# jklebes/MetropolisEngine

Hardware: AMD Instinct MI355X
Metric: MC steps/sec (chains x sweeps) at 2^20 chains, 16 params (higher is better)
Workload: dtype f64

## Files before the change

metropolisengine_amd/csrc/me_device.h:

```cpp
#pragma once

#include <type_traits>
#include <utility>

#include <hip/hip_runtime.h>
#include <stdint.h>

#include "me_internal.h"
#include "me_math64.h"

namespace me {

struct U4 {
  uint32_t x, y, z, w;
};

__device__ __forceinline__ uint32_t xor3(uint32_t a, uint32_t b, uint32_t c) {
  return __builtin_amdgcn_bitop3_b32(a, b, c, 0x96);
}
__device__ __forceinline__ U4 philox4x32_10(U4 c, uint32_t k0, uint32_t k1) {
#pragma unroll
  for (int r = 0; r < 10; ++r) {
    const uint64_t p0 = (uint64_t)0xD2511F53u * c.x;
    const uint64_t p1 = (uint64_t)0xCD9E8D57u * c.z;
    U4 n;
    n.x = xor3((uint32_t)(p1 >> 32), c.y, k0);
    n.y = (uint32_t)p1;
    n.z = xor3((uint32_t)(p0 >> 32), c.w, k1);
    n.w = (uint32_t)p0;
    c = n;
    k0 += 0x9E3779B9u;
    k1 += 0xBB67AE85u;
  }
  return c;
}
__device__ __forceinline__ U4 philox_counter(unsigned long long gid, unsigned long long step, int b) {
  U4 ctr;
  ctr.x = (uint32_t)gid;
  ctr.y = (uint32_t)(gid >> 32);
  ctr.z = (uint32_t)step;
  ctr.w = ((uint32_t)(step >> 32) << 16) | (uint32_t)b;
  return ctr;
}
__device__ __forceinline__ U4 philox_block(unsigned long long gid, unsigned long long step, int b, uint32_t seed_lo, uint32_t seed_hi) {
  return philox4x32_10(philox_counter(gid, step, b), seed_lo, seed_hi);
}

__device__ __forceinline__ float fma_(float a, float b, float c) { return __builtin_fmaf(a, b, c); }
__device__ __forceinline__ double fma_(double a, double b, double c) { return __builtin_fma(a, b, c); }

template <typename R>
struct Num;

template <>
struct Num<float> {
  static __device__ __forceinline__ void prepare() {}
  static __device__ __forceinline__ float unit(uint32_t w) {
    return __builtin_fmaf((float)w, 2.3283064365386963e-10f, 1.1641532182693481e-10f);
  }
  static __device__ __forceinline__ void normal_pair(uint32_t wa, uint32_t wb, float &g0, float &g1) {
    const float u1 = unit(wa), u2 = unit(wb);
    const float r = __builtin_amdgcn_sqrtf(-1.3862943611198906f * __builtin_amdgcn_logf(u1));
    g0 = r * __builtin_amdgcn_cosf(u2);
    g1 = r * __builtin_amdgcn_sinf(u2);
  }
  static __device__ __forceinline__ bool uphill(float u, float d, float, float inv_temp_log2e) {
    return u <= __builtin_amdgcn_exp2f(-d * inv_temp_log2e);
  }
  static __device__ __forceinline__ float adapt(float w, bool acc, float ratio, float p, float damping,
                                                float up, float down) {
    return __builtin_fmaf(w, acc ? up : down, w);
  }
  static __device__ __forceinline__ float sqrt_(float v) { return __builtin_sqrtf(v); }
  static __device__ __forceinline__ float abs_(float v) { return __builtin_fabsf(v); }
  static __device__ __forceinline__ bool finite(float v) { return __builtin_isfinite(v); }
};

template <>
struct Num<double> {
  static __device__ __forceinline__ double (*log_table())[2] {
    __shared__ __attribute__((aligned(16))) double table[math64::kLogEntries][2];
    return table;
  }
  static __device__ __forceinline__ void prepare() {
    double(*table)[2] = log_table();
    for (int k0 = threadIdx.x; k0 < math64::kLogEntries; k0 += 2 * (int)blockDim.x) {
      const int k1 = k0 + (int)blockDim.x;
      const bool second = k1 < math64::kLogEntries;
      const double a0 = math64::kLogTable[k0][0], a1 = math64::kLogTable[k0][1];
      const double b0 = second ? math64::kLogTable[k1][0] : 0.0, b1 = second ? math64::kLogTable[k1][1] : 0.0;
      table[k0][0] = a0;
      table[k0][1] = a1;
      if (second) {
        table[k1][0] = b0;
        table[k1][1] = b1;
      }
    }
    __syncthreads();
  }
  static __device__ __forceinline__ double unit(uint32_t w) { return ((double)w + 0.5) * (1.0 / 4294967296.0); }
  static __device__ __forceinline__ void normal_pair(uint32_t wa, uint32_t wb, double &g0, double &g1) {
    math64::normal_pair(wa, wb, log_table(), g0, g1);
  }
  static __device__ __forceinline__ bool uphill(double u, double d, double inv_temp, double) {
    return u <= math64::exp_nonpos(-d * inv_temp);
  }
  static __device__ __forceinline__ double adapt(double w, bool acc, double ratio, double p, double damping,
                                                 double, double) {
    const double scale = w * ratio;
    return acc ? w + scale * (1.0 - p) / damping : w - scale * p / damping;
  }
  static __device__ __forceinline__ double sqrt_(double v) { return sqrt(v); }
  static __device__ __forceinline__ double abs_(double v) { return fabs(v); }
  static __device__ __forceinline__ bool finite(double v) { return isfinite(v); }
};

#ifndef ME_NT_AUX
#define ME_NT_AUX 2
#endif
template <typename R>
struct Field {
  __amdgpu_buffer_rsrc_t rsrc;
  unsigned int row_bytes;
  __device__ __forceinline__ Field(const R *base, long long n, int rows)
      : rsrc(__builtin_amdgcn_make_buffer_rsrc(const_cast<R *>(base), 0, (unsigned int)(rows * n * (long long)sizeof(R)),
                                               0x00020000)),
        row_bytes((unsigned int)(n * (long long)sizeof(R))) {}
  __device__ __forceinline__ R load(int row, unsigned int chain_off) const {
    if constexpr (sizeof(R) == 4) {
      return __builtin_bit_cast(R, __builtin_amdgcn_raw_buffer_load_b32(rsrc, chain_off, (unsigned int)row * row_bytes, 0));
    } else {
      const auto v = __builtin_amdgcn_raw_buffer_load_b64(rsrc, chain_off, (unsigned int)row * row_bytes, 0);
      return __builtin_bit_cast(R, v);
    }
  }
  __device__ __forceinline__ R load_nt(int row, unsigned int chain_off) const {
    if constexpr (sizeof(R) == 4) {
      return __builtin_bit_cast(R, __builtin_amdgcn_raw_buffer_load_b32(rsrc, chain_off, (unsigned int)row * row_bytes, ME_NT_AUX));
    } else {
      const auto v = __builtin_amdgcn_raw_buffer_load_b64(rsrc, chain_off, (unsigned int)row * row_bytes, ME_NT_AUX);
      return __builtin_bit_cast(R, v);
    }
  }
  __device__ __forceinline__ void store_nt(int row, unsigned int chain_off, R value) const {
    if constexpr (sizeof(R) == 4) {
      __builtin_amdgcn_raw_buffer_store_b32(__builtin_bit_cast(unsigned int, value), rsrc, chain_off,
                                            (unsigned int)row * row_bytes, ME_NT_AUX);
    } else {
      using v2 = decltype(__builtin_amdgcn_raw_buffer_load_b64(rsrc, 0u, 0u, 0));
      __builtin_amdgcn_raw_buffer_store_b64(__builtin_bit_cast(v2, value), rsrc, chain_off,
                                            (unsigned int)row * row_bytes, ME_NT_AUX);
    }
  }
  __device__ __forceinline__ void store(int row, unsigned int chain_off, R value) const {
    if constexpr (sizeof(R) == 4) {
      __builtin_amdgcn_raw_buffer_store_b32(__builtin_bit_cast(unsigned int, value), rsrc, chain_off,
                                            (unsigned int)row * row_bytes, 0);
    } else {
      using v2 = decltype(__builtin_amdgcn_raw_buffer_load_b64(rsrc, 0u, 0u, 0));
      __builtin_amdgcn_raw_buffer_store_b64(__builtin_bit_cast(v2, value), rsrc, chain_off,
                                            (unsigned int)row * row_bytes, 0);
    }
  }
};

template <typename R>
__device__ __forceinline__ R chain_energy(const Field<R> &fe, unsigned int chain_off, int n_terms) {
  R e = fe.load(0, chain_off);
  for (int t = 1; t < n_terms; ++t) e = e + fe.load(t, chain_off);
  return e;
}

template <typename R>
__device__ __forceinline__ unsigned int tiled_offset(long long c, int entries) {
  return (unsigned int)(((c >> 6) * (long long)entries * 64 + (c & 63)) * (long long)sizeof(R));
}
template <typename R>
struct TiledField {
  __amdgpu_buffer_rsrc_t rsrc;
  __device__ __forceinline__ TiledField(const R *base, long long n, int entries)
      : rsrc(__builtin_amdgcn_make_buffer_rsrc(const_cast<R *>(base), 0,
                                               (unsigned int)(((n + 63) >> 6) * (long long)entries * 64 * (long long)sizeof(R)),
                                               0x00020000)) {}
  static constexpr unsigned int kEntryBytes = 64u * (unsigned int)sizeof(R);
  template <int AUX>
  __device__ __forceinline__ R load_aux(int k, unsigned int tile_off) const {
    if constexpr (sizeof(R) == 4) {
      return __builtin_bit_cast(R, __builtin_amdgcn_raw_buffer_load_b32(rsrc, tile_off, (unsigned int)k * kEntryBytes, AUX));
    } else {
      const auto v = __builtin_amdgcn_raw_buffer_load_b64(rsrc, tile_off, (unsigned int)k * kEntryBytes, AUX);
      return __builtin_bit_cast(R, v);
    }
  }
  template <int AUX>
  __device__ __forceinline__ void store_aux(int k, unsigned int tile_off, R value) const {
    if constexpr (sizeof(R) == 4) {
      __builtin_amdgcn_raw_buffer_store_b32(__builtin_bit_cast(unsigned int, value), rsrc, tile_off, (unsigned int)k * kEntryBytes, AUX);
    } else {
      using v2 = decltype(__builtin_amdgcn_raw_buffer_load_b64(rsrc, 0u, 0u, 0));
      __builtin_amdgcn_raw_buffer_store_b64(__builtin_bit_cast(v2, value), rsrc, tile_off, (unsigned int)k * kEntryBytes, AUX);
    }
  }
  __device__ __forceinline__ R load(int k, unsigned int tile_off) const { return load_aux<0>(k, tile_off); }
  __device__ __forceinline__ R load_nt(int k, unsigned int tile_off) const { return load_aux<ME_NT_AUX>(k, tile_off); }
  __device__ __forceinline__ void store(int k, unsigned int tile_off, R value) const { store_aux<0>(k, tile_off, value); }
  __device__ __forceinline__ void store_nt(int k, unsigned int tile_off, R value) const { store_aux<ME_NT_AUX>(k, tile_off, value); }
};

template <bool NT, class F>
__device__ __forceinline__ auto packed_load(const F &f, int row, unsigned int chain_off) {
  if constexpr (NT) return f.load_nt(row, chain_off);
  else return f.load(row, chain_off);
}
template <bool NT, class F, typename R>
__device__ __forceinline__ void packed_store(const F &f, int row, unsigned int chain_off, R value) {
  if constexpr (NT) f.store_nt(row, chain_off, value);
  else f.store(row, chain_off, value);
}

template <typename R, bool NTS>
struct StateField : Field<R> {
  using Field<R>::Field;
  __device__ __forceinline__ R load(int row, unsigned int chain_off) const {
    if constexpr (NTS) return Field<R>::load_nt(row, chain_off);
    else return Field<R>::load(row, chain_off);
  }
  __device__ __forceinline__ void store(int row, unsigned int chain_off, R value) const {
    if constexpr (NTS) Field<R>::store_nt(row, chain_off, value);
    else Field<R>::store(row, chain_off, value);
  }
};

#ifndef ME_TILED_STATE_DOF
#define ME_TILED_STATE_DOF 16
#endif
constexpr int kTiledStateDof = ME_TILED_STATE_DOF;
template <typename R, int D, bool NTS = false>
struct XField {
  static constexpr bool kTiled = D >= kTiledStateDof;
  std::conditional_t<kTiled, TiledField<R>, StateField<R, NTS>> f;
  __device__ __forceinline__ XField(const R *base, long long n) : f(base, n, D) {}
  static __device__ __forceinline__ unsigned int offset(long long c) {
    if constexpr (kTiled) return tiled_offset<R>(c, D);
    else return (unsigned int)c * (unsigned int)sizeof(R);
  }
  __device__ __forceinline__ R load(int row, unsigned int off) const {
    if constexpr (kTiled && NTS) return f.load_nt(row, off);
    else return f.load(row, off);
  }
  __device__ __forceinline__ void store(int row, unsigned int off, R value) const {
    if constexpr (kTiled && NTS) f.store_nt(row, off, value);
    else f.store(row, off, value);
  }
};
template <typename R, int D>
__device__ __forceinline__ long long state_index(long long c, int row, long long n) {
  if constexpr (D >= kTiledStateDof) return ((c >> 6) * (long long)D + row) * 64 + (c & 63);
  else return (long long)row * n + c;
}

constexpr int kMaxPackedInRegisters = 160;
#ifndef ME_STREAM_F64_ENTRIES
#define ME_STREAM_F64_ENTRIES 96
#endif
constexpr int kStreamF64Entries = ME_STREAM_F64_ENTRIES;

template <typename R, int NR, int NC>
struct EnergyIso {
  static constexpr int D = NR + 2 * NC;
  R a;
  __device__ __forceinline__ R operator()(const R (&x)[D]) const {
    R s0 = 0, s1 = 0;
#pragma unroll
    for (int d = 0; d + 1 < D; d += 2) {
      s0 += x[d] * x[d];
      s1 += x[d + 1] * x[d + 1];
    }
    if constexpr (D % 2 == 1) s0 += x[D - 1] * x[D - 1];
    return a * (s0 + s1);
  }
};

template <typename R, int NR, int NC>
struct EnergyDiag {
  static constexpr int D = NR + 2 * NC;
  R w[D];
  __device__ __forceinline__ R operator()(const R (&x)[D]) const {
    R s0 = 0, s1 = 0;
#pragma unroll
    for (int d = 0; d + 1 < D; d += 2) {
      s0 += w[d] * x[d] * x[d];
      s1 += w[d + 1] * x[d + 1] * x[d + 1];
    }
    if constexpr (D % 2 == 1) s0 += w[D - 1] * x[D - 1] * x[D - 1];
    return s0 + s1;
  }
};

template <typename R, int NR, int NC>
struct EnergyDense {
  static constexpr int D = NR + 2 * NC;
  static constexpr int PT = D * (D + 1) / 2;
  const R *a;
  static __device__ __forceinline__ R *folded() {
    __shared__ R t[PT];
    return t;
  }
  __device__ __forceinline__ void prepare() const {
    R *t = folded();
    constexpr int kBatch = 8;
    for (int k0 = threadIdx.x; k0 < PT; k0 += kBatch * (int)blockDim.x) {
      R lo[kBatch], hi[kBatch];
#pragma unroll
      for (int u = 0; u < kBatch; ++u) {
        const int k = k0 + u * (int)blockDim.x;
        lo[u] = hi[u] = R(0);
        if (k < PT) {
          int i = (int)((__builtin_sqrtf((float)(8 * k + 1)) - 1.0f) * 0.5f);
          if ((i + 1) * (i + 2) / 2 <= k) ++i;
          if (i * (i + 1) / 2 > k) --i;
          const int j = k - i * (i + 1) / 2;
          lo[u] = a[i * D + j];
          if (i != j) hi[u] = a[j * D + i];
        }
      }
#pragma unroll
      for (int u = 0; u < kBatch; ++u) {
        const int k = k0 + u * (int)blockDim.x;
        if (k < PT) t[k] = lo[u] + hi[u];
      }
    }
    __syncthreads();
  }
  __device__ __forceinline__ R operator()(const R (&x)[D]) const {
    const R *t = folded();
    asm volatile("" ::: "memory");
    R e = 0;
#pragma unroll
    for (int i = 0; i < D; ++i) {
      R y = 0;
#pragma unroll
      for (int j = 0; j <= i; ++j) y += t[i * (i + 1) / 2 + j] * x[j];
      e += x[i] * y;
    }
    return e;
  }
};

template <typename R, int NR, int NC>
struct EnergyLandau {
  static constexpr int D = NR + 2 * NC;
  R k, alpha, beta;
  __device__ __forceinline__ R operator()(const R (&x)[D]) const {
    static_assert(NR == 2 && NC == 1, "Landau toy is 2 real + 1 complex");
    const R a2 = fma_(x[2], x[2], x[3] * x[3]);
    const R ox = R(1) - x[0], oy = R(1) - x[1];
    return fma_(x[0] * x[1], fma_(beta * a2, a2, alpha * a2), fma_(k * ox, ox, k * oy * oy));
  }
};

template <typename R, int NR, int NC>
struct EnergyCylinder {
  static constexpr int D = NR + 2 * NC;
  R kappa, gamma, wavenumber;
  __device__ __forceinline__ R operator()(const R (&x)[D]) const {
    static_assert(NR >= 1 && NC >= 1, "cylinder surrogate needs an amplitude and a field");
    R s = 0;
#pragma unroll
    for (int i = 0; i < NR; ++i) s += x[i] * x[i];
    const R x0 = x[0];
    const R surface = kappa * s / (R(1) - x0 * x0);
    const R amp = R(1) + R(0.5) * x0 * x0;
    R field = 0, tot = 0;
#pragma unroll
    for (int j = 0; j < NC; ++j) {
      const R q = wavenumber * (R(j) - R(NC - 1) * R(0.5));
      const R mod2 = fma_(x[NR + j], x[NR + j], x[NR + NC + j] * x[NR + NC + j]);
      field += (gamma + q * q * amp) * mod2;
      tot += mod2;
    }
    return surface + field + R(0.5) * tot * tot;
  }
};

template <typename R, int NR, int NC>
struct EnergyLandauTerms {
  static constexpr int D = NR + 2 * NC;
  static constexpr int kTerms = 2;
  R k, alpha, beta;
  static constexpr unsigned term_groups(int t) { return t == 0 ? 3u : 1u; }
  __device__ __forceinline__ R term(int t, const R (&x)[D]) const {
    static_assert(NR == 2 && NC == 1, "Landau toy is 2 real + 1 complex");
    if (t == 0) {
      const R a2 = fma_(x[2], x[2], x[3] * x[3]);
      return x[0] * x[1] * fma_(beta * a2, a2, alpha * a2);
    }
    const R ox = R(1) - x[0], oy = R(1) - x[1];
    return fma_(k * ox, ox, k * oy * oy);
  }
};

template <class E, typename R, int D>
__device__ __forceinline__ auto energy_reject(const E &en, const R (&x)[D], int) -> decltype(en.reject(x)) {
  return en.reject(x);
}
template <class E, typename R, int D>
__device__ __forceinline__ bool energy_reject(const E &, const R (&)[D], long) {
  return false;
}

template <class E>
__device__ __forceinline__ auto energy_prepare(const E &en, int) -> decltype(en.prepare()) {
  en.prepare();
}
template <class E>
__device__ __forceinline__ void energy_prepare(const E &, long) {}

template <class E, class = void>
struct term_count { static constexpr int value = 1; };
template <class E>
struct term_count<E, std::void_t<decltype(E::kTerms)>> { static constexpr int value = E::kTerms; };

template <typename R, class Energy, int GROUP>
struct EnergyLedger {
  static constexpr int T = term_count<Energy>::value;
  R term[T];
  static constexpr bool moves(int t) {
    if constexpr (T == 1 || GROUP == GROUP_ALL) return true;
    else return (Energy::term_groups(t) & (GROUP == GROUP_REAL ? 1u : 2u)) != 0u;
  }
  template <class F>
  __device__ __forceinline__ void load(const F &fe, unsigned int coff) {
#pragma unroll
    for (int t = 0; t < T; ++t)
      if (moves(t)) term[t] = fe.load(t, coff);
  }
  template <class F>
  __device__ __forceinline__ void store(const F &fe, unsigned int coff) const {
#pragma unroll
    for (int t = 0; t < T; ++t)
      if (moves(t)) fe.store(t, coff, term[t]);
  }
  __device__ __forceinline__ R partial() const {
    R s = 0;
    bool first = true;
#pragma unroll
    for (int t = 0; t < T; ++t)
      if (moves(t)) {
        s = first ? term[t] : s + term[t];
        first = false;
      }
    return s;
  }
  template <int D>
  __device__ __forceinline__ R propose(const Energy &en, const R (&xp)[D], R (&out)[T]) const {
    if constexpr (T == 1) {
      out[0] = en(xp);
      return out[0];
    } else {
      R s = 0;
      bool first = true;
#pragma unroll
      for (int t = 0; t < T; ++t)
        if (moves(t)) {
          out[t] = en.term(t, xp);
          s = first ? out[t] : s + out[t];
          first = false;
        }
      return s;
    }
  }
  __device__ __forceinline__ void commit(bool accept, const R (&out)[T]) {
#pragma unroll
    for (int t = 0; t < T; ++t)
      if (moves(t)) term[t] = accept ? out[t] : term[t];
  }
};

template <typename R>
struct StepArgs {
  R *x, *energy, *width;
  const R *factor;
  const R *inj_normals;
  const R *inj_uniforms;
  unsigned long long *accept_slots;
  unsigned int *status;
  long long n;
  unsigned long long chain_offset, step_index;
  uint32_t seed_lo, seed_hi;
  int n_sweeps, reject_kind;
  int split_widths;
  int stale_total;
  R reject_bound, temp, inv_temp, inv_temp_log2e, ratio, p, damping, up, down;
  const R *ladder;
  int tiles_per_rung;
};

template <typename R>
StepArgs<R> typed(const StepLaunch &l) {
  StepArgs<R> a;
  a.x = (R *)l.x;
  a.energy = (R *)l.energy;
  a.width = (R *)l.width;
  a.factor = (const R *)l.factor;
  a.inj_normals = (const R *)l.inj_normals;
  a.inj_uniforms = (const R *)l.inj_uniforms;
  a.accept_slots = l.accept_slots;
  a.status = l.status;
  a.n = l.n;
  a.chain_offset = l.chain_offset;
  a.step_index = l.step_index;
  a.seed_lo = (uint32_t)l.seed;
  a.seed_hi = (uint32_t)(l.seed >> 32);
  a.n_sweeps = l.n_sweeps;
  a.reject_kind = l.reject_kind;
  a.split_widths = l.split_widths;
  a.stale_total = l.stale_total;
  a.reject_bound = (R)l.reject_bound;
  a.temp = (R)l.temp;
  a.inv_temp = l.temp > 0 ? (R)(1.0 / l.temp) : (R)0;
  a.inv_temp_log2e = l.temp > 0 ? (R)(1.4426950408889634 / l.temp) : (R)0;
  a.ratio = (R)l.ratio;
  a.p = (R)l.target_acceptance;
  a.damping = (R)l.damping;
  a.up = (R)(l.ratio * (1.0 - l.target_acceptance) / l.damping);
  a.down = (R)(-l.ratio * l.target_acceptance / l.damping);
  a.ladder = (const R *)l.ladder;
  a.tiles_per_rung = l.tiles_per_rung;
  return a;
}

template <typename R>
__device__ __forceinline__ void publish_step(const StepArgs<R> &a, unsigned int waves, unsigned int wave_accepted, bool bad_energy,
                                             bool bad_width, bool bad_pivot = false) {
  if ((threadIdx.x & 63) == 0 && wave_accepted) {
    unsigned long long *slot = a.accept_slots + (size_t)blockIdx.x * waves + (threadIdx.x >> 6);
    *slot += (unsigned long long)wave_accepted;
  }
  const unsigned int bits = (bad_energy ? ST_NONFINITE_ENERGY : 0u) | (bad_width ? ST_BAD_WIDTH : 0u) | (bad_pivot ? ST_BAD_PIVOT : 0u);
  if (bits) atomicOr(a.status, bits);
}

template <bool LADDER, typename R>
__device__ __forceinline__ bool uphill_at(const StepArgs<R> &a, long long c, R u, R diff) {
  if constexpr (!LADDER) {
    return a.temp > R(0) && Num<R>::uphill(u, diff, a.inv_temp, a.inv_temp_log2e);
  } else {
    const int rung = __builtin_amdgcn_readfirstlane((int)(c >> 6)) / a.tiles_per_rung;
    return Num<R>::uphill(u, diff, a.ladder[2 * rung], a.ladder[2 * rung + 1]);
  }
}

__host__ __device__ constexpr int tri(int i, int j) { return i * (i + 1) / 2 + j; }
__host__ __device__ constexpr int cre(int pr, int i, int j) { return pr + i * i + 2 * j; }
__host__ __device__ constexpr int cim(int pr, int i, int j) { return pr + i * i + 2 * j + 1; }
__host__ __device__ constexpr int cdiag(int pr, int i) { return pr + i * i + 2 * i; }

template <class F, int... I>
__device__ __forceinline__ void static_for_impl(F &&fn, std::integer_sequence<int, I...>) {
  (fn(std::integral_constant<int, I>{}), ...);
}
template <int N, class F>
__device__ __forceinline__ void static_for(F &&fn) {
  static_for_impl(fn, std::make_integer_sequence<int, N>{});
}
__host__ __device__ constexpr unsigned long long join_halves(int hi, int lo) {
  return ((unsigned long long)(unsigned int)hi << 32) | (unsigned long long)(unsigned int)lo;
}
static_assert(join_halves(0x00007f12, (int)0x80000000u) == 0x00007f1280000000ull, "low half with bit 31 set must not sign-extend");
static_assert(join_halves((int)0xffff8000u, (int)0xfffffff0u) == 0xffff8000fffffff0ull, "both halves are zero-extended");
#ifndef ME_STREAM_CHUNK_BYTES
#define ME_STREAM_CHUNK_BYTES 128
#endif

template <typename R, int NR, int NC, bool INJECT>
__device__ __forceinline__ void draw_step(const StepArgs<R> &a, long long c, unsigned long long gid, int s,
                                          R (&g)[2 * ((NR + 2 * NC + 1) / 2)], R &u) {
  constexpr int D = NR + 2 * NC;
  constexpr int NW = 2 * ((D + 1) / 2);
  constexpr int NBLK = (NW + 1 + 3) / 4;
  using N_ = Num<R>;
  [[maybe_unused]] const unsigned long long step = a.step_index + (unsigned long long)s;
  if constexpr (INJECT) {
#pragma unroll
    for (int j = 0; j < D; ++j) g[j] = a.inj_normals[((long long)s * D + j) * a.n + c];
    u = a.inj_uniforms[(long long)s * a.n + c];
  } else {
    uint32_t words[4 * NBLK];
#pragma unroll
    for (int b = 0; b < NBLK; ++b) {
      const U4 o = philox_block(gid, step, b, a.seed_lo, a.seed_hi);
      words[4 * b + 0] = o.x;
      words[4 * b + 1] = o.y;
      words[4 * b + 2] = o.z;
      words[4 * b + 3] = o.w;
    }
#pragma unroll
    for (int q = 0; q < NW / 2; ++q) N_::normal_pair(words[2 * q], words[2 * q + 1], g[2 * q], g[2 * q + 1]);
    u = N_::unit(words[NW]);
  }

}

template <typename R, int NR, int NC, int CK, int GROUP, class Fac>
__device__ __forceinline__ void propose_registers(const R (&x)[NR + 2 * NC], const R (&g)[2 * ((NR + 2 * NC + 1) / 2)], R w_r, R w_c,
                                                  Fac &&fac, R (&xp)[NR + 2 * NC]) {
  constexpr int D = NR + 2 * NC;
  [[maybe_unused]] constexpr int PR = NR * (NR + 1) / 2;
  constexpr bool MOVE_REAL = NR > 0 && GROUP != GROUP_COMPLEX;
  constexpr bool MOVE_COMPLEX = NC > 0 && GROUP != GROUP_REAL;
#pragma unroll
  for (int d = 0; d < D; ++d) xp[d] = x[d];
  if constexpr (CK == CK_IDENTITY) {
    if constexpr (MOVE_REAL) {
#pragma unroll
      for (int i = 0; i < NR; ++i) xp[i] = x[i] + w_r * g[i];
    }
    if constexpr (MOVE_COMPLEX) {
#pragma unroll
      for (int j = 0; j < NC; ++j) {
        xp[NR + j] = x[NR + j] + w_c * (g[NR + j] * R(0.70710678118654752440));
        xp[NR + NC + j] = x[NR + NC + j] + w_c * (g[NR + NC + j] * R(0.70710678118654752440));
      }
    }
  } else {
    if constexpr (MOVE_REAL) {
#pragma unroll
      for (int i = 0; i < NR; ++i) {
        R acc = 0;
#pragma unroll
        for (int j = 0; j <= i; ++j) acc += fac(tri(i, j)) * g[j];
        xp[i] = x[i] + w_r * acc;
      }
    }
    if constexpr (MOVE_COMPLEX) {
#pragma unroll
      for (int i = 0; i < NC; ++i) {
        R are = 0, aim = 0;
#pragma unroll
        for (int j = 0; j < i; ++j) {
          const R lre = fac(cre(PR, i, j));
          const R lim = fac(cim(PR, i, j));
          const R wre = g[NR + j] * R(0.70710678118654752440), wim = g[NR + NC + j] * R(0.70710678118654752440);
          are += lre * wre - lim * wim;
          aim += lre * wim + lim * wre;
        }
        const R ld = fac(cdiag(PR, i));
        are += ld * (g[NR + i] * R(0.70710678118654752440));
        aim += ld * (g[NR + NC + i] * R(0.70710678118654752440));
        xp[NR + i] = x[NR + i] + w_c * are;
        xp[NR + NC + i] = x[NR + NC + i] + w_c * aim;
      }
    }
  }

}

template <typename R, int NR, int NC, class Energy, int CK, int GROUP, bool LADDER, class Ledger>
__device__ __forceinline__ void decide_step(const StepArgs<R> &a, long long c, const Energy &en, bool stale_total, R u,
                                            const R (&g)[2 * ((NR + 2 * NC + 1) / 2)], R (&x)[NR + 2 * NC], const R (&xp)[NR + 2 * NC],
                                            Ledger &ledger, R &total_q5, R &w, R &w_r, R &w_c, unsigned int &wave_accepted,
                                            bool &bad_energy) {
  [[maybe_unused]] constexpr int D = NR + 2 * NC;
  constexpr bool MOVE_REAL = NR > 0 && GROUP != GROUP_COMPLEX;
  constexpr bool MOVE_COMPLEX = NC > 0 && GROUP != GROUP_REAL;
  using N_ = Num<R>;
  bool rejected = false;
  if (a.reject_kind == ME_REJECT_ABS_REAL0_GE) rejected = !(N_::abs_(xp[0]) < a.reject_bound);
  else if (a.reject_kind == ME_REJECT_USER) rejected = energy_reject(en, xp, 0);
  R terms_new[Ledger::T];
  const R e_new = ledger.propose(en, xp, terms_new);
  const R diff = e_new - (stale_total ? total_q5 : ledger.partial());
  bool accept = diff <= R(0);
  if constexpr (LADDER) accept = accept || uphill_at<true>(a, c, u, diff);
  else if (a.temp > R(0)) accept = accept || N_::uphill(u, diff, a.inv_temp, a.inv_temp_log2e);
  accept = accept && !rejected;
  bad_energy |= (!rejected && !N_::finite(e_new));
  if constexpr (CK == CK_IDENTITY) {
    const R wa_r = accept ? w_r : R(0), wa_c = accept ? w_c : R(0);
    if constexpr (MOVE_REAL) {
#pragma unroll
      for (int i = 0; i < NR; ++i) x[i] = x[i] + wa_r * g[i];
    }
    if constexpr (MOVE_COMPLEX) {
#pragma unroll
      for (int j = 0; j < NC; ++j) {
        x[NR + j] = x[NR + j] + wa_c * (g[NR + j] * R(0.70710678118654752440));
        x[NR + NC + j] = x[NR + NC + j] + wa_c * (g[NR + NC + j] * R(0.70710678118654752440));
      }
    }
  } else {
#pragma unroll
    for (int d = 0; d < D; ++d) x[d] = accept ? xp[d] : x[d];
  }
  if (stale_total) total_q5 = accept ? e_new : total_q5;
  else ledger.commit(accept, terms_new);
  w = N_::adapt(w, accept, a.ratio, a.p, a.damping, a.up, a.down);
  if constexpr (GROUP == GROUP_ALL) w_r = w_c = w;
  else if constexpr (GROUP == GROUP_REAL) w_r = w;
  else w_c = w;
  wave_accepted += (unsigned int)__popcll(__ballot(accept));
}

template <typename R, int NR, int NC, class Energy, int CK, bool INJECT, int GROUP, bool LADDER, class Ledger, class Fac>
__device__ __forceinline__ void run_sweeps(const StepArgs<R> &a, const Energy &en, long long c, unsigned long long gid,
                                           bool stale_total, R (&x)[NR + 2 * NC], Ledger &ledger, R &total_q5, R &w, R &w_r,
                                           R &w_c, Fac &&fac, unsigned int &wave_accepted, bool &bad_energy) {
  constexpr int D = NR + 2 * NC;
  constexpr int NW = 2 * ((D + 1) / 2);
  for (int s = 0; s < a.n_sweeps; ++s) {
    R g[NW], u, xp[D];
    draw_step<R, NR, NC, INJECT>(a, c, gid, s, g, u);
    propose_registers<R, NR, NC, CK, GROUP>(x, g, w_r, w_c, fac, xp);
    decide_step<R, NR, NC, Energy, CK, GROUP, LADDER>(a, c, en, stale_total, u, g, x, xp, ledger, total_q5, w, w_r, w_c, wave_accepted, bad_energy);
  }
}

#ifndef ME_STEP_WAVES_PER_EU
#define ME_STEP_WAVES_PER_EU 0
#endif
#if ME_STEP_WAVES_PER_EU > 0
#define ME_STEP_BOUNDS __launch_bounds__(kFusedStepThreads, ME_STEP_WAVES_PER_EU)
#else
#define ME_STEP_BOUNDS __launch_bounds__(kFusedStepThreads)
#endif

#ifndef ME_STEP_PRIO_SHIFT
#define ME_STEP_PRIO_SHIFT 8
#endif
__device__ __forceinline__ void stagger_priority() {
#if ME_STEP_PRIO_SHIFT >= 0
  switch ((blockIdx.x >> ME_STEP_PRIO_SHIFT) & 3u) {
    case 0: __builtin_amdgcn_s_setprio(3); break;
    case 1: __builtin_amdgcn_s_setprio(2); break;
    case 2: __builtin_amdgcn_s_setprio(1); break;
    default: break;
  }
#endif
}

template <typename R, int NR, int NC, class Energy, int CK, bool INJECT = false, int GROUP = GROUP_ALL, bool NTS = false,
          bool LADDER = false>
__global__ void ME_STEP_BOUNDS k_step(StepArgs<R> a, Energy en) {
  constexpr int D = NR + 2 * NC;
  constexpr bool MIXED = NR > 0 && NC > 0;
  static_assert(GROUP == GROUP_ALL || MIXED, "group-wise kernels exist for mixed engines only");
  using N_ = Num<R>;

  stagger_priority();
  if constexpr (!INJECT) N_::prepare();
  energy_prepare(en, 0);
  unsigned int wave_accepted = 0;
  bool bad_energy = false, bad_width = false;
  const long long stride = (long long)gridDim.x * blockDim.x;
  using Ledger = EnergyLedger<R, Energy, GROUP>;
  const XField<R, D, NTS> fx(a.x, a.n);
  const StateField<R, NTS> fe(a.energy, a.n, Ledger::T + (MIXED ? 1 : 0)), fw(a.width, a.n, MIXED ? 3 : 1);
  const bool stale_total = MIXED && GROUP == GROUP_ALL && a.stale_total != 0;
  constexpr bool PER_CHAIN = CK == CK_PER_CHAIN || CK == CK_PER_CHAIN_NT;
  constexpr int PF = PER_CHAIN ? NR * (NR + 1) / 2 + NC * NC : 0;
  constexpr bool STREAM_FACTOR = PER_CHAIN && (PF > kMaxPackedInRegisters ||
                                               (!INJECT && sizeof(R) == 8 && NC == 0 && PF > kStreamF64Entries));
  const TiledField<R> ffac(a.factor, a.n, STREAM_FACTOR ? 0 : PF);
  for (long long c = (long long)blockIdx.x * blockDim.x + threadIdx.x; c < a.n; c += stride) {
    const unsigned int coff = (unsigned int)c * (unsigned int)sizeof(R);
    const unsigned int xoff = fx.offset(c);
    R x[D];
#pragma unroll
    for (int d = 0; d < D; ++d) x[d] = fx.load(d, xoff);
    Ledger ledger;
    R total_q5 = R(0);
    if (stale_total) total_q5 = fe.load(Ledger::T, coff);
    else ledger.load(fe, coff);
    R w = fw.load(MIXED ? GROUP : 0, coff);
    R w_r = w, w_c = w;
    if constexpr (MIXED && GROUP == GROUP_ALL) {
      if (a.split_widths) {
        w_r = fw.load(GROUP_REAL, coff);
        w_c = fw.load(GROUP_COMPLEX, coff);
      }
    }
    const unsigned long long gid = a.chain_offset + (unsigned long long)c;
    [[maybe_unused]] const unsigned int toff = tiled_offset<R>(c, PF);
    auto fac = [&](int k) -> R {
      if constexpr (CK == CK_PER_CHAIN_NT) return ffac.load_nt(k, toff);
      else if constexpr (CK == CK_PER_CHAIN) return ffac.load(k, toff);
      else return a.factor[k];
    };

    if constexpr (STREAM_FACTOR) {
      constexpr int NW = 2 * ((D + 1) / 2);
      for (int s = 0; s < a.n_sweeps; ++s) {
        static_assert(!INJECT, "the streamed-factor form has no replay hook");
        constexpr int NBLK = (NW + 1 + 3) / 4;
        const unsigned long long step = a.step_index + (unsigned long long)s;
        R g[NW];
        R u_accept;
        {
          uint32_t words[4 * NBLK];
#pragma unroll
          for (int b = 0; b < NBLK; ++b) {
            const U4 o = philox_block(gid, step, b, a.seed_lo, a.seed_hi);
            words[4 * b + 0] = o.x;
            words[4 * b + 1] = o.y;
            words[4 * b + 2] = o.z;
            words[4 * b + 3] = o.w;
          }
#pragma unroll
          for (int q = 0; q < NW / 2; ++q) N_::normal_pair(words[2 * q], words[2 * q + 1], g[2 * q], g[2 * q + 1]);
          u_accept = N_::unit(words[NW]);
        }
        R xp[D];
#pragma unroll
        for (int d = 0; d < D; ++d) xp[d] = x[d];
        asm volatile("" ::: "memory");
        constexpr int CH = (int)(ME_STREAM_CHUNK_BYTES / sizeof(R));
        const R *tile_base = a.factor + (c >> 6) * (long long)PF * 64;
        const unsigned long long tb = (unsigned long long)tile_base;
        const R *tile_uniform = (const R *)join_halves(__builtin_amdgcn_readfirstlane((int)(tb >> 32)),
                                                       __builtin_amdgcn_readfirstlane((int)(unsigned int)tb));
        const __amdgpu_buffer_rsrc_t tile = __builtin_amdgcn_make_buffer_rsrc(const_cast<R *>(tile_uniform), 0,
                                                                               (unsigned int)(PF * 64 * sizeof(R)), 0x00020000);
        const unsigned int lane_off = (unsigned int)(c & 63) * (unsigned int)sizeof(R);
        auto entry = [&](int k) -> R {
          constexpr int AUX = CK == CK_PER_CHAIN_NT ? ME_NT_AUX : 0;
          if constexpr (sizeof(R) == 4)
            return __builtin_bit_cast(R, __builtin_amdgcn_raw_buffer_load_b32(tile, lane_off, (unsigned int)k * 64u * 4u, AUX));
          else
            return __builtin_bit_cast(R, __builtin_amdgcn_raw_buffer_load_b64(tile, lane_off, (unsigned int)k * 64u * 8u, AUX));
        };
        R f[2][CH];
#pragma unroll
        for (int u = 0; u < CH; ++u)
          if (u < PF) f[0][u] = entry(u);
        auto use = [&](auto entry_index) -> R {
          constexpr int k = decltype(entry_index)::value;
          if constexpr (k % CH == 0) {
            __builtin_amdgcn_sched_barrier(0);
#pragma unroll
            for (int u = 0; u < CH; ++u)
              if (k + CH + u < PF) f[(k / CH + 1) & 1][u] = entry(k + CH + u);
            __builtin_amdgcn_sched_barrier(0);
          }
          return f[(k / CH) & 1][k % CH];
        };
        static_for<NR>([&](auto row_index) {
          constexpr int i = decltype(row_index)::value;
          R acc = 0;
          static_for<i + 1>([&](auto col_index) {
            constexpr int j = decltype(col_index)::value, k = tri(i, j);
            const R l = use(std::integral_constant<int, k>{});
            acc = j == 0 ? l * g[0] : acc + l * g[j];
          });
          if constexpr (GROUP != GROUP_COMPLEX) xp[i] = x[i] + w_r * acc;
        });
        static_for<NC>([&](auto row_index) {
          constexpr int i = decltype(row_index)::value;
          R are = 0, aim = 0;
          static_for<i>([&](auto col_index) {
            constexpr int j = decltype(col_index)::value;
            const R lre = use(std::integral_constant<int, cre(NR * (NR + 1) / 2, i, j)>{});
            const R lim = use(std::integral_constant<int, cim(NR * (NR + 1) / 2, i, j)>{});
            const R wre = g[NR + j] * R(0.70710678118654752440), wim = g[NR + NC + j] * R(0.70710678118654752440);
            are += lre * wre - lim * wim;
            aim += lre * wim + lim * wre;
          });
          const R ld = use(std::integral_constant<int, cdiag(NR * (NR + 1) / 2, i)>{});
          are += ld * (g[NR + i] * R(0.70710678118654752440));
          aim += ld * (g[NR + NC + i] * R(0.70710678118654752440));
          if constexpr (GROUP != GROUP_REAL) {
            xp[NR + i] = x[NR + i] + w_c * are;
            xp[NR + NC + i] = x[NR + NC + i] + w_c * aim;
          }
        });
        bool rejected = false;
        if (a.reject_kind == ME_REJECT_ABS_REAL0_GE) rejected = !(N_::abs_(xp[0]) < a.reject_bound);
        else if (a.reject_kind == ME_REJECT_USER) rejected = energy_reject(en, xp, 0);
        R terms_new[Ledger::T];
        const R e_new = ledger.propose(en, xp, terms_new);
        const R diff = e_new - (stale_total ? total_q5 : ledger.partial());
        bool accept = diff <= R(0);
        if constexpr (LADDER) accept = accept || uphill_at<true>(a, c, u_accept, diff);
        else if (a.temp > R(0)) accept = accept || N_::uphill(u_accept, diff, a.inv_temp, a.inv_temp_log2e);
        accept = accept && !rejected;
        bad_energy |= (!rejected && !N_::finite(e_new));
#pragma unroll
        for (int d = 0; d < D; ++d) x[d] = accept ? xp[d] : x[d];
        if (stale_total) total_q5 = accept ? e_new : total_q5;
        else ledger.commit(accept, terms_new);
        w = N_::adapt(w, accept, a.ratio, a.p, a.damping, a.up, a.down);
        if constexpr (GROUP == GROUP_ALL) w_r = w_c = w;
        else if constexpr (GROUP == GROUP_REAL) w_r = w;
        else w_c = w;
        wave_accepted += (unsigned int)__popcll(__ballot(accept));
      }
    } else {
      run_sweeps<R, NR, NC, Energy, CK, INJECT, GROUP, LADDER>(a, en, c, gid, stale_total, x, ledger, total_q5, w, w_r, w_c, fac, wave_accepted, bad_energy);
    }
    bad_width |= !(w > R(0));
#pragma unroll
    for (int d = 0; d < D; ++d) fx.store(d, xoff, x[d]);
    if (stale_total) fe.store(Ledger::T, coff, total_q5);
    else ledger.store(fe, coff);
    fw.store(MIXED ? GROUP : 0, coff, w);
  }
  publish_step(a, blockDim.x >> 6, wave_accepted, bad_energy, bad_width);
}

template <typename R, int NR, int NC, class Energy>
__global__ void __launch_bounds__(kStepThreads) k_init_energy(const R *xs, R *energy, long long n, unsigned int *status,
                                                                Energy en, int total_row) {
  constexpr int D = NR + 2 * NC;
  energy_prepare(en, 0);
  const long long stride = (long long)gridDim.x * kStepThreads;
  for (long long c = (long long)blockIdx.x * kStepThreads + threadIdx.x; c < n; c += stride) {
    R x[D];
#pragma unroll
    for (int d = 0; d < D; ++d) x[d] = xs[state_index<R, D>(c, d, n)];
    constexpr int T = term_count<Energy>::value;
    bool finite = true;
    R total = R(0);
#pragma unroll
    for (int t = 0; t < T; ++t) {
      R e;
      if constexpr (T == 1) e = en(x);
      else e = en.term(t, x);
      energy[(long long)t * n + c] = e;
      total = t == 0 ? e : total + e;
      finite = finite && Num<R>::finite(e);
    }
    if (total_row >= 0) energy[(long long)total_row * n + c] = total;
    if (!finite) atomicOr(status, (unsigned int)ST_NONFINITE_ENERGY);
  }
}

}
#include "me_packed_walk.h"
namespace me {

template <typename R>
struct MeasureArgs {
  const R *x, *width;
  R *mean, *cov, *obs_mean, *factor;
  unsigned int *status;
  long long n;
  R keep;
  R inv_i;
  R cov_keep;
  int update_cov, write_factor, split_widths;
};

template <typename R>
MeasureArgs<R> typed_measure(const MeasureLaunch &l) {
  MeasureArgs<R> a;
  a.x = (const R *)l.x;
  a.width = (const R *)l.width;
  a.mean = (R *)l.mean;
  a.cov = (R *)l.cov;
  a.obs_mean = (R *)l.obs_mean;
  a.factor = (R *)l.factor;
  a.status = l.status;
  a.n = l.n;
  const double i = (double)l.measure_count;
  a.keep = (R)((i - 1.0) / i);
  a.inv_i = (R)(1.0 / i);
  a.cov_keep = (R)((i - 2.0) / (i - 1.0));
  a.update_cov = l.update_cov;
  a.split_widths = l.split_widths;
  a.write_factor = l.write_factor;
  return a;
}

template <typename R, int NR, int NC>
__device__ __forceinline__ void cholesky_packed(R (&m)[NR * (NR + 1) / 2 + NC * NC], bool &bad_pivot) {
  constexpr int PR = NR * (NR + 1) / 2;
  using N_ = Num<R>;
#pragma unroll
    for (int j = 0; j < NR; ++j) {
      R s = m[tri(j, j)];
#pragma unroll
      for (int k = 0; k < j; ++k) s = fma_(-m[tri(j, k)], m[tri(j, k)], s);
      if (!(s > R(0))) { bad_pivot = true; s = R(1e-30); }
      const R dg = N_::sqrt_(s);
      const R inv = R(1) / dg;
      m[tri(j, j)] = dg;
#pragma unroll
      for (int i = j + 1; i < NR; ++i) {
        R t = m[tri(i, j)];
#pragma unroll
        for (int k = 0; k < j; ++k) t = fma_(-m[tri(i, k)], m[tri(j, k)], t);
        m[tri(i, j)] = t * inv;
      }
    }
#pragma unroll
    for (int j = 0; j < NC; ++j) {
      R s = m[cdiag(PR, j)];
#pragma unroll
      for (int k = 0; k < j; ++k) s = fma_(-m[cim(PR, j, k)], m[cim(PR, j, k)], fma_(-m[cre(PR, j, k)], m[cre(PR, j, k)], s));
      if (!(s > R(0))) { bad_pivot = true; s = R(1e-30); }
      const R dg = N_::sqrt_(s);
      const R inv = R(1) / dg;
      m[cdiag(PR, j)] = dg;
#pragma unroll
      for (int i = j + 1; i < NC; ++i) {
        R tr = m[cre(PR, i, j)], ti = m[cim(PR, i, j)];
#pragma unroll
        for (int k = 0; k < j; ++k) {
          const R ar = m[cre(PR, i, k)], ai2 = m[cim(PR, i, k)];
          const R br = m[cre(PR, j, k)], bi2 = m[cim(PR, j, k)];
          tr = fma_(-ai2, bi2, fma_(-ar, br, tr));
          ti = fma_(ar, bi2, fma_(-ai2, br, ti));
        }
        m[cre(PR, i, j)] = tr * inv;
        m[cim(PR, i, j)] = ti * inv;
      }
    }
}

#ifndef ME_MEASURE_WAVES
#define ME_MEASURE_WAVES 1
#endif

template <typename R, int NR, int NC, bool PER_CHAIN_COV, bool FUSED, bool NT, bool NTM, class WidthFn>
__device__ __forceinline__ void measure_chain(const MeasureArgs<R> &a, long long c, const R (&x)[NR + 2 * NC],
                                              const Field<R> &fmean, const Field<R> &fobs, const TiledField<R> &fcov,
                                              const TiledField<R> &ffac, [[maybe_unused]] R (*s_delta)[kStepThreads],
                                              WidthFn &&widths, bool &bad_pivot) {
  constexpr int D = NR + 2 * NC;
  constexpr int PR = NR * (NR + 1) / 2;
  constexpr int P = PR + NC * NC;
  constexpr int NOBS = 2 * NR + NC;
  constexpr bool STREAM = PER_CHAIN_COV && P > kMaxPackedInRegisters;
  using N_ = Num<R>;
  const unsigned int coff = (unsigned int)c * (unsigned int)sizeof(R);
  [[maybe_unused]] const unsigned int toff = tiled_offset<R>(c, P);
  R delta[D];
  {
    R mu[D];
#pragma unroll
    for (int d = 0; d < D; ++d) mu[d] = packed_load<NTM>(fmean, d, coff);
#pragma unroll
    for (int d = 0; d < D; ++d) {
      if constexpr (STREAM) s_delta[d][threadIdx.x] = x[d] - mu[d];
      else delta[d] = x[d] - mu[d];
      packed_store<NTM>(fmean, d, coff, fma_(x[d], a.inv_i, mu[d] * a.keep));
    }
  }
  constexpr int kBatch = 32;
#pragma unroll
  for (int k0 = 0; k0 < NOBS; k0 += kBatch) {
    R m[kBatch];
#pragma unroll
    for (int u = 0; u < kBatch; ++u)
      if (k0 + u < NOBS) m[u] = packed_load<NTM>(fobs, k0 + u, coff);
#pragma unroll
    for (int u = 0; u < kBatch; ++u) {
      const int k = k0 + u;
      if (k < NOBS) {
        R o;
        if (k < NR) o = N_::abs_(x[k]);
        else if (k < NR + NC) o = N_::sqrt_(fma_(x[k], x[k], x[k + NC] * x[k + NC]));
        else o = x[k - NR - NC] * x[k - NR - NC];
        packed_store<NTM>(fobs, k, coff, fma_(o, a.inv_i, m[u] * a.keep));
      }
    }
  }
  if constexpr (PER_CHAIN_COV) {
    if (a.update_cov) {
      R w_real, w_cplx;
      widths(w_real, w_cplx);
      const R w2_real = w_real * w_real, w2_cplx = w_cplx * w_cplx;
      if constexpr (STREAM) {
        covariance_walk(a.cov + (c >> 6) * (long long)P * 64 + (c & 63), s_delta, NR, NC, (int)threadIdx.x, a.inv_i, a.cov_keep,
                        w2_real, w2_cplx);
      } else {
      R m[P];
#pragma unroll
      for (int k = 0; k < P; ++k) m[k] = packed_load<NT>(fcov, k, toff);
#pragma unroll
      for (int i = 0; i < NR; ++i)
#pragma unroll
        for (int j = 0; j <= i; ++j) {
          const int k = tri(i, j);
          R v = fma_(delta[i] * delta[j], a.inv_i, m[k] * a.cov_keep);
          if (i == j) v = fma_(w2_real, a.inv_i, v);
          packed_store<NT>(fcov, k, toff, v);
          m[k] = v;
        }
#pragma unroll
      for (int i = 0; i < NC; ++i) {
        const R ai = delta[NR + i], bi = delta[NR + NC + i];
#pragma unroll
        for (int j = 0; j < i; ++j) {
          const R aj = delta[NR + j], bj = delta[NR + NC + j];
          const int kr = cre(PR, i, j), ki = cim(PR, i, j);
          const R vr = fma_(fma_(ai, aj, bi * bj), a.inv_i, m[kr] * a.cov_keep);
          const R vi = fma_(fma_(bi, aj, -(ai * bj)), a.inv_i, m[ki] * a.cov_keep);
          packed_store<NT>(fcov, kr, toff, vr);
          packed_store<NT>(fcov, ki, toff, vi);
          m[kr] = vr;
          m[ki] = -vi;
        }
        const int kd = cdiag(PR, i);
        const R vd = fma_(w2_cplx, a.inv_i, fma_(fma_(ai, ai, bi * bi), a.inv_i, m[kd] * a.cov_keep));
        packed_store<NT>(fcov, kd, toff, vd);
        m[kd] = vd;
      }
      if constexpr (FUSED) {
        if (a.write_factor) {
          cholesky_packed<R, NR, NC>(m, bad_pivot);
#pragma unroll
          for (int k = 0; k < P; ++k) packed_store<NT>(ffac, k, toff, m[k]);
        }
      }
      }
    }
  }
}

template <typename R, int NR, int NC, bool PER_CHAIN_COV, bool FUSED, bool NT, bool NTM>
__global__ void __launch_bounds__(kStepThreads, ME_MEASURE_WAVES) k_measure(MeasureArgs<R> a) {
  constexpr int D = NR + 2 * NC;
  constexpr int P = NR * (NR + 1) / 2 + NC * NC;
  constexpr int NOBS = 2 * NR + NC;
  bool bad_pivot = false;
  const long long stride = (long long)gridDim.x * kStepThreads;
  const XField<R, D> fx(a.x, a.n);
  const Field<R> fw(a.width, a.n, (NR > 0 && NC > 0) ? 3 : 1), fmean(a.mean, a.n, D), fobs(a.obs_mean, a.n, NOBS);
  constexpr bool STREAM = PER_CHAIN_COV && P > kMaxPackedInRegisters;
  const TiledField<R> fcov(a.cov, a.n, (PER_CHAIN_COV && !STREAM) ? P : 0);
  const TiledField<R> ffac(a.factor, a.n, (PER_CHAIN_COV && FUSED) ? P : 0);
  __shared__ R s_delta[STREAM ? D : 1][kStepThreads];
  for (long long c = (long long)blockIdx.x * kStepThreads + threadIdx.x; c < a.n; c += stride) {
    const unsigned int coff = (unsigned int)c * (unsigned int)sizeof(R);
    const unsigned int xoff = fx.offset(c);
    R x[D];
#pragma unroll
    for (int d = 0; d < D; ++d) x[d] = fx.load(d, xoff);
    measure_chain<R, NR, NC, PER_CHAIN_COV, FUSED, NT, NTM>(a, c, x, fmean, fobs, fcov, ffac, s_delta, [&](R &w_real, R &w_cplx) {
      constexpr bool MIXED = NR > 0 && NC > 0;
      w_real = fw.load((MIXED && a.split_widths) ? 1 : 0, coff);
      w_cplx = fw.load((MIXED && a.split_widths) ? 2 : 0, coff);
    }, bad_pivot);
  }
  if (bad_pivot) atomicOr(a.status, (unsigned int)ST_BAD_PIVOT);
}

template <typename R, int NR, int NC, class Energy, int CK, bool NT, bool NTM, bool LADDER = false>
__global__ void ME_STEP_BOUNDS k_cycle(StepArgs<R> a, MeasureArgs<R> ma, Energy en) {
  constexpr int D = NR + 2 * NC;
  constexpr int P = NR * (NR + 1) / 2 + NC * NC;
  constexpr int NOBS = 2 * NR + NC;
  constexpr bool MIXED = NR > 0 && NC > 0;
  static_assert(P <= kMaxPackedInRegisters, "k_cycle keeps the packed matrix in registers");
  static_assert(CK == CK_IDENTITY || CK == CK_SHARED || CK == CK_PER_CHAIN, "NT selects the non-temporal factor read");
  constexpr int CKX = CK == CK_PER_CHAIN ? (NT ? CK_PER_CHAIN_NT : CK_PER_CHAIN) : CK;
  using N_ = Num<R>;
  N_::prepare();
  energy_prepare(en, 0);
  unsigned int wave_accepted = 0;
  bool bad_energy = false, bad_width = false, bad_pivot = false;
  const long long stride = (long long)gridDim.x * blockDim.x;
  using Ledger = EnergyLedger<R, Energy, GROUP_ALL>;
  const XField<R, D> fx(a.x, a.n);
  const Field<R> fe(a.energy, a.n, Ledger::T + (MIXED ? 1 : 0)), fw(a.width, a.n, MIXED ? 3 : 1);
  const Field<R> fmean(ma.mean, a.n, D), fobs(ma.obs_mean, a.n, NOBS);
  const TiledField<R> fcov(ma.cov, a.n, P), ffac(ma.factor, a.n, P);
  const bool stale_total = MIXED && a.stale_total != 0;
  for (long long c = (long long)blockIdx.x * blockDim.x + threadIdx.x; c < a.n; c += stride) {
    const unsigned int coff = (unsigned int)c * (unsigned int)sizeof(R);
    const unsigned int xoff = fx.offset(c);
    R x[D];
#pragma unroll
    for (int d = 0; d < D; ++d) x[d] = fx.load(d, xoff);
    Ledger ledger;
    R total_q5 = R(0);
    if (stale_total) total_q5 = fe.load(Ledger::T, coff);
    else ledger.load(fe, coff);
    R w = fw.load(0, coff);
    R w_r = w, w_c = w;
    if constexpr (MIXED) {
      if (a.split_widths) {
        w_r = fw.load(GROUP_REAL, coff);
        w_c = fw.load(GROUP_COMPLEX, coff);
      }
    }
    const unsigned long long gid = a.chain_offset + (unsigned long long)c;
    [[maybe_unused]] const unsigned int toff = tiled_offset<R>(c, P);
    auto fac = [&](int k) -> R {
      if constexpr (CK == CK_PER_CHAIN) return packed_load<NT>(ffac, k, toff);
      else return a.factor[k];
    };
    run_sweeps<R, NR, NC, Energy, CKX, false, GROUP_ALL, LADDER>(a, en, c, gid, stale_total, x, ledger, total_q5, w, w_r, w_c, fac,
                                                         wave_accepted, bad_energy);
    bad_width |= !(w > R(0));
#pragma unroll
    for (int d = 0; d < D; ++d) fx.store(d, xoff, x[d]);
    if (stale_total) fe.store(Ledger::T, coff, total_q5);
    else ledger.store(fe, coff);
    fw.store(0, coff, w);
    measure_chain<R, NR, NC, true, true, NT, NTM>(ma, c, x, fmean, fobs, fcov, ffac, nullptr,
                                                  [&](R &w_real, R &w_cplx) { w_real = w_cplx = w; }, bad_pivot);
  }
  publish_step(a, blockDim.x >> 6, wave_accepted, bad_energy, bad_width, bad_pivot);
}

template <typename R, int NR, bool NT>
__global__ void __launch_bounds__(kStepThreads) k_factor_stream(const R *cov, R *factor, unsigned int *status, long long n) {
  constexpr int P = NR * (NR + 1) / 2;
  constexpr int ROWS = sizeof(R) == 4 ? 4 : 2;
  __shared__ R rows[ROWS * NR][kStepThreads];
  bool bad_pivot = false;
  const long long stride = (long long)gridDim.x * kStepThreads;
  for (long long c = (long long)blockIdx.x * kStepThreads + threadIdx.x; c < n; c += stride) {
    const long long base = (c >> 6) * (long long)P * 64 + (c & 63);
    factor_real_rows<R, ROWS, NT>(cov + base, factor + base, NR, rows, (int)threadIdx.x, bad_pivot);
  }
  if (bad_pivot) atomicOr(status, (unsigned int)ST_BAD_PIVOT);
}

template <typename R, int NR, int NC, bool NT>
__global__ void __launch_bounds__(kStepThreads) k_factor_mixed(const R *cov, R *factor, unsigned int *status, long long n) {
  constexpr int PR = NR * (NR + 1) / 2, P = PR + NC * NC;
  using N_ = Num<R>;
  bool bad_pivot = false;
  const long long stride = (long long)gridDim.x * kStepThreads;
  for (long long c = (long long)blockIdx.x * kStepThreads + threadIdx.x; c < n; c += stride) {
    const long long base = (c >> 6) * (long long)P * 64 + (c & 63);
    const R *cv = cov + base;
    R *fc = factor + base;
    auto in = [&](int k) -> R { return NT ? __builtin_nontemporal_load(cv + (long long)k * 64) : cv[(long long)k * 64]; };
    for (int i = 0; i < NR; ++i)
      for (int j = 0; j <= i; ++j) {
        R s = in(tri(i, j));
        for (int k = 0; k < j; ++k) s = fma_(-fc[(long long)tri(i, k) * 64], fc[(long long)tri(j, k) * 64], s);
        if (j < i) {
          fc[(long long)tri(i, j) * 64] = s / fc[(long long)tri(j, j) * 64];
        } else {
          if (!(s > R(0))) { bad_pivot = true; s = R(1e-30); }
          fc[(long long)tri(i, i) * 64] = N_::sqrt_(s);
        }
      }
    factor_complex_rows<R, NT>(cv, fc, PR, NC, bad_pivot);
  }
  if (bad_pivot) atomicOr(status, (unsigned int)ST_BAD_PIVOT);
}

}
```

Baseline: 19.30 billion.

## Overlap log-table staging and first chain-state load, prefetch next chain state

Splits the f64 log-table setup into a global-load request and an LDS commit, so the first chain's state loads are issued before the table is written to shared memory and the barrier is taken. Inside the grid-stride loop, the next chain's state is loaded after the current chain's stores. The aim is to hide global load latency behind the table setup and the barrier. It also rewrites the width adaptation to use a single division. The costs are extra live registers for the prefetched state (x, ledger, widths), which may lower occupancy, and a redundant clamped load for threads that have no chain.

```diff
diff --git a/metropolisengine_amd/csrc/me_device.h b/metropolisengine_amd/csrc/me_device.h
--- a/metropolisengine_amd/csrc/me_device.h
+++ b/metropolisengine_amd/csrc/me_device.h
@@ -54,7 +54,10 @@
 
 template <>
 struct Num<float> {
+  struct LogRows {};
   static __device__ __forceinline__ void prepare() {}
+  static __device__ __forceinline__ LogRows request_table() { return {}; }
+  static __device__ __forceinline__ void commit_table(const LogRows &) {}
   static __device__ __forceinline__ float unit(uint32_t w) {
     return __builtin_fmaf((float)w, 2.3283064365386963e-10f, 1.1641532182693481e-10f);
   }
@@ -82,22 +85,25 @@
     __shared__ __attribute__((aligned(16))) double table[math64::kLogEntries][2];
     return table;
   }
-  static __device__ __forceinline__ void prepare() {
+  static_assert(2 * kStepThreads >= math64::kLogEntries, "two rows per thread must cover the log table in the smallest step block");
+  struct LogRows {
+    double a0, a1, b0, b1;
+  };
+  static __device__ __forceinline__ int table_row(unsigned int k) { return (int)min(k, (unsigned int)(math64::kLogEntries - 1)); }
+  static __device__ __forceinline__ LogRows request_table() {
+    const int k0 = table_row(threadIdx.x), k1 = table_row(threadIdx.x + blockDim.x);
+    return {math64::kLogTable[k0][0], math64::kLogTable[k0][1], math64::kLogTable[k1][0], math64::kLogTable[k1][1]};
+  }
+  static __device__ __forceinline__ void commit_table(const LogRows &rows) {
     double(*table)[2] = log_table();
-    for (int k0 = threadIdx.x; k0 < math64::kLogEntries; k0 += 2 * (int)blockDim.x) {
-      const int k1 = k0 + (int)blockDim.x;
-      const bool second = k1 < math64::kLogEntries;
-      const double a0 = math64::kLogTable[k0][0], a1 = math64::kLogTable[k0][1];
-      const double b0 = second ? math64::kLogTable[k1][0] : 0.0, b1 = second ? math64::kLogTable[k1][1] : 0.0;
-      table[k0][0] = a0;
-      table[k0][1] = a1;
-      if (second) {
-        table[k1][0] = b0;
-        table[k1][1] = b1;
-      }
-    }
+    const int k0 = table_row(threadIdx.x), k1 = table_row(threadIdx.x + blockDim.x);
+    table[k0][0] = rows.a0;
+    table[k0][1] = rows.a1;
+    table[k1][0] = rows.b0;
+    table[k1][1] = rows.b1;
     __syncthreads();
   }
+  static __device__ __forceinline__ void prepare() { commit_table(request_table()); }
   static __device__ __forceinline__ double unit(uint32_t w) { return ((double)w + 0.5) * (1.0 / 4294967296.0); }
   static __device__ __forceinline__ void normal_pair(uint32_t wa, uint32_t wb, double &g0, double &g1) {
     math64::normal_pair(wa, wb, log_table(), g0, g1);
@@ -108,7 +114,8 @@
   static __device__ __forceinline__ double adapt(double w, bool acc, double ratio, double p, double damping,
                                                  double, double) {
     const double scale = w * ratio;
-    return acc ? w + scale * (1.0 - p) / damping : w - scale * p / damping;
+    const double delta = (acc ? scale * (1.0 - p) : scale * p) / damping;
+    return acc ? w + delta : w - delta;
   }
   static __device__ __forceinline__ double sqrt_(double v) { return sqrt(v); }
   static __device__ __forceinline__ double abs_(double v) { return fabs(v); }
@@ -415,6 +422,10 @@
 }
 template <class E>
 __device__ __forceinline__ void energy_prepare(const E &, long) {}
+template <class E, class = void>
+struct stages_lds : std::false_type {};
+template <class E>
+struct stages_lds<E, std::void_t<decltype(std::declval<const E &>().prepare())>> : std::true_type {};
 
 template <class E, class = void>
 struct term_count { static constexpr int value = 1; };
@@ -719,6 +730,9 @@
 #ifndef ME_STEP_WAVES_PER_EU
 #define ME_STEP_WAVES_PER_EU 0
 #endif
+#ifndef ME_STEP_SPLIT_TABLE
+#define ME_STEP_SPLIT_TABLE 1
+#endif
 #if ME_STEP_WAVES_PER_EU > 0
 #define ME_STEP_BOUNDS __launch_bounds__(kFusedStepThreads, ME_STEP_WAVES_PER_EU)
 #else
@@ -748,7 +762,10 @@
   using N_ = Num<R>;
 
   stagger_priority();
-  if constexpr (!INJECT) N_::prepare();
+  constexpr bool SPLIT_TABLE = ME_STEP_SPLIT_TABLE && !INJECT && sizeof(R) == 8 && !stages_lds<Energy>::value;
+  [[maybe_unused]] typename N_::LogRows log_rows;
+  if constexpr (SPLIT_TABLE) log_rows = N_::request_table();
+  else if constexpr (!INJECT) N_::prepare();
   energy_prepare(en, 0);
   unsigned int wave_accepted = 0;
   bool bad_energy = false, bad_width = false;
@@ -762,23 +779,51 @@
   constexpr bool STREAM_FACTOR = PER_CHAIN && (PF > kMaxPackedInRegisters ||
                                                (!INJECT && sizeof(R) == 8 && NC == 0 && PF > kStreamF64Entries));
   const TiledField<R> ffac(a.factor, a.n, STREAM_FACTOR ? 0 : PF);
-  for (long long c = (long long)blockIdx.x * blockDim.x + threadIdx.x; c < a.n; c += stride) {
-    const unsigned int coff = (unsigned int)c * (unsigned int)sizeof(R);
-    const unsigned int xoff = fx.offset(c);
-    R x[D];
+  auto load_state = [&](long long chain, unsigned int &coff, unsigned int &xoff, R (&x)[D], Ledger &ledger, R &total_q5, R &w,
+                        R &w_r, R &w_c) {
+    coff = (unsigned int)chain * (unsigned int)sizeof(R);
+    xoff = fx.offset(chain);
 #pragma unroll
     for (int d = 0; d < D; ++d) x[d] = fx.load(d, xoff);
-    Ledger ledger;
-    R total_q5 = R(0);
     if (stale_total) total_q5 = fe.load(Ledger::T, coff);
     else ledger.load(fe, coff);
-    R w = fw.load(MIXED ? GROUP : 0, coff);
-    R w_r = w, w_c = w;
+    w = fw.load(MIXED ? GROUP : 0, coff);
+    w_r = w_c = w;
     if constexpr (MIXED && GROUP == GROUP_ALL) {
       if (a.split_widths) {
         w_r = fw.load(GROUP_REAL, coff);
         w_c = fw.load(GROUP_COMPLEX, coff);
       }
+    }
+  };
+  struct {
+    unsigned int coff, xoff;
+    R x[D];
+    Ledger ledger;
+    R total_q5, w, w_r, w_c;
+  } next{};
+  const long long first = (long long)blockIdx.x * blockDim.x + threadIdx.x;
+  if constexpr (SPLIT_TABLE) {
+    load_state(first < a.n ? first : a.n - 1, next.coff, next.xoff, next.x, next.ledger, next.total_q5, next.w, next.w_r, next.w_c);
+    N_::commit_table(log_rows);
+  }
+  for (long long c = first; c < a.n; c += stride) {
+    unsigned int coff, xoff;
+    R x[D];
+    Ledger ledger;
+    R total_q5 = R(0), w, w_r, w_c;
+    if constexpr (SPLIT_TABLE) {
+      coff = next.coff;
+      xoff = next.xoff;
+#pragma unroll
+      for (int d = 0; d < D; ++d) x[d] = next.x[d];
+      ledger = next.ledger;
+      total_q5 = next.total_q5;
+      w = next.w;
+      w_r = next.w_r;
+      w_c = next.w_c;
+    } else {
+      load_state(c, coff, xoff, x, ledger, total_q5, w, w_r, w_c);
     }
     const unsigned long long gid = a.chain_offset + (unsigned long long)c;
     [[maybe_unused]] const unsigned int toff = tiled_offset<R>(c, PF);
@@ -903,6 +948,10 @@
     if (stale_total) fe.store(Ledger::T, coff, total_q5);
     else ledger.store(fe, coff);
     fw.store(MIXED ? GROUP : 0, coff, w);
+    if constexpr (SPLIT_TABLE) {
+      if (c + stride < a.n)
+        load_state(c + stride, next.coff, next.xoff, next.x, next.ledger, next.total_q5, next.w, next.w_r, next.w_c);
+    }
   }
   publish_step(a, blockDim.x >> 6, wave_accepted, bad_energy, bad_width);
 }
```

After: 19.71 billion, median of 6. 1.02x the previous value.
